# yhg926/MetaKSSD

Hardware: AMD Instinct MI355X
Metric: Gbases/s sketched (150 bp synthetic reads, L3K11 -A) (higher is better)
Workload: dtype u64 k-mers over u8 bases (integer)

## Files before the change

### metakssd_amd/csrc/mk_engine.hip

```cpp
#include "metakssd_hip.h"
#include "mk_poison.hip.h"
#include "mk_kernels.hip.h"
#include "mk_stream.hip.h"
#include "mk_fastq_long.hip.h"
#include "mk_batch.hip.h"
#include "mk_gz.hip.h"
#include "mk_packed.hip.h"

#include <math.h>
#include <stdarg.h>
#include <stdio.h>
#include <stdlib.h>
#include <string.h>

#include <vector>

static thread_local char g_create_error[512] = "";

struct mk_evpair { hipEvent_t a, b; };
#define MK_TICKETS 16
#define MK_REGIONS 3
#define MK_REGION_BYTES ((size_t)256 << 20)

struct mk_engine {
// ... 796 lines not shown
  if (e->tail_active) {
    if (e->split_stream && e->stream == e->own_stream) {
      MK_HIP(e, hipEventRecord(e->ev_scan_pre, e->own_stream));
      MK_HIP(e, hipStreamWaitEvent(e->split_stream, e->ev_scan_pre, 0));
      e->stream = e->split_stream;
    }
    e->tail_active = false;
  }
  return MK_OK;
}

extern "C" int mk_sketch_begin_occ(mk_engine *e, int min_occurrence) {
  if (!e) return MK_ERR_ARG;
  if (min_occurrence < 1 || min_occurrence >= 15)
    return mk_fail(e, MK_ERR_ARG, "fastq2co(): Occurence num should be 1..14 (got %d)", min_occurrence);
  int rc = mk_sketch_begin(e, MK_MODE_OCC_SET);
  if (rc == MK_OK) e->min_occ = (uint32_t)min_occurrence;
  return rc;
}

extern "C" int mk_sketch_begin(mk_engine *e, int mode) {
  if (!e) return MK_ERR_ARG;
  const bool tail = (mode & MK_BEGIN_NOTHING_FOLLOWS) != 0;
  mode &= ~MK_BEGIN_NOTHING_FOLLOWS;
  if (mode < MK_MODE_KOC || mode > MK_MODE_OCC_SET) return MK_ERR_ARG;
  MK_HIP(e, hipSetDevice(e->device));
  { int rc = mk_tables_alloc(e); if (rc) return rc; }
  { int rc = mk_tail_end(e); if (rc) return rc; }
  e->tail = tail && e->scan_stream && e->stream == e->split_stream;
  { int rc = mk_poison_scratch(e); if (rc) return rc; }
  mk_evpair ev{};
  if (e->profiling) { ev = mk_ev_get(e); MK_HIP(e, hipEventRecord(ev.a, e->stream)); }
  bool clear_front = false;
  if (e->sparse && e->tables_tracked) {
    if (!e->tab.fr || e->big_maybe_dirty) {
      hipLaunchKernelGGL(mk_dirty_list_kernel, dim3(1), dim3(1024), 0, e->stream, e->d_dirty_acc, e->acc_words, e->d_list_acc, e->d_nlist, 1,
                         (const uint32_t *)nullptr);
      hipLaunchKernelGGL(mk_dirty_clear_kernel, dim3((unsigned)e->num_cu * 8u), dim3(256), 0, e->stream, e->tab.kc, e->tab.ordinv, e->kp.S,
                         (const uint32_t *)e->d_list_acc, (const uint32_t *)e->d_nlist, (uint32_t)MK_SPARSE_SHIFT, (uint32_t *)nullptr,
                         (const uint32_t *)nullptr, (const uint32_t *)nullptr, (uint32_t)MK_DUMP_SHIFT);
      MK_HIP(e, hipGetLastError());
    }
    if (e->tab.fr) { clear_front = true; e->big_maybe_dirty = false; }
    if (!e->slot_clean) {
      MK_HIP(e, hipMemsetAsync(e->d_slot, 0xFF, (size_t)e->kp.S * sizeof(uint32_t), e->stream));
      e->slot_clean = true;
    }
  } else {
    if (!e->tab.fr || e->big_maybe_dirty) MK_HIP(e, hipMemsetAsync(e->d_tab, 0, e->tab_bytes, e->stream));
    if (e->tab.fr) { clear_front = true; e->big_maybe_dirty = false; }
    if (e->sparse) {
      MK_HIP(e, hipMemsetAsync(e->d_slot, 0xFF, (size_t)e->kp.S * sizeof(uint32_t), e->stream));
      MK_HIP(e, hipMemsetAsync(e->d_dirty_acc, 0, (size_t)e->acc_words * 4, e->stream));
      MK_HIP(e, hipMemsetAsync(e->d_dirty_slot, 0, (size_t)e->slot_words * 4, e->stream));
      e->tables_tracked = true;
      e->slot_clean = true;
    }
  }
  {
    const unsigned long long n16 = clear_front ? (unsigned long long)e->front_slots : 0ull;
    unsigned long long blocks = (n16 + 1023u) / 1024u;
    if (blocks > (unsigned long long)e->num_cu * 8u) blocks = (unsigned long long)e->num_cu * 8u;
    if (blocks == 0) blocks = 1;
    const bool fa = e->fa_used && e->d_fa_state;
    hipLaunchKernelGGL(mk_begin_clear_kernel, dim3((unsigned)blocks), dim3(256), 0, e->stream, (uint4 *)e->d_front, n16, e->d_counters,
                       (uint32_t *)e->d_fa_state, fa ? (uint32_t)(sizeof(mk_fa_state) / 4u) : 0u);
    MK_HIP(e, hipGetLastError());
    e->counter0_used = false;
  }
  if (e->profiling) { MK_HIP(e, hipEventRecord(ev.b, e->stream)); e->ev_clear.push_back(ev); }
  e->region_open = false;
  e->mode = mode;
  e->min_occ = 1;
  e->begun = true;
  e->compacted = false;
  e->count_queued = false;
  e->D = 0;
  e->fa_used = false; e->fa_final = false; e->fa_tail = 0; e->fa_rows_done = 0; e->fa_pitch = 0;
  e->fq_used = false; e->fq_pending = false; e->fq_carry_len = 0; e->fq_total = 0; e->fq_timed = false; e->fq_frame_ms = 0;
  return MK_OK;
}

template <int K, int SK, bool V, int T, int NP, bool OP>
static hipError_t mk_launch_scan_t(mk_engine *e, const mk_scan_args &a, dim3 grid, size_t lds, hipStream_t s) {
  const void *fn = (const void *)mk_scan_kernel<K, SK, V, T, NP, OP>;
  size_t *granted = nullptr;
  for (auto &g : e->lds_granted) if (g.first == fn) granted = &g.second;
  if (!granted) { e->lds_granted.emplace_back(fn, 0); granted = &e->lds_granted.back().second; }
  if (lds > *granted) {
    hipError_t r = hipFuncSetAttribute(fn, hipFuncAttributeMaxDynamicSharedMemorySize, (int)lds);
    if (r != hipSuccess) return r;
    *granted = lds;
  }
  hipLaunchKernelGGL((mk_scan_kernel<K, SK, V, T, NP, OP>), grid, dim3(T), lds, s, a);
  return hipGetLastError();
}
template <int K, int SK, bool V>
static hipError_t mk_launch_scan_k(mk_engine *e, int threads, bool onepass, const mk_scan_args &a, dim3 grid, size_t lds, hipStream_t s) {
  constexpr int NPBIG = V ? MK_MAX_PIECES : MK_MAX_CB / 4;
  constexpr int NPSMALL = V ? 5 : 20;
  const bool small = a.ppr <= (uint32_t)NPSMALL;
  if constexpr (V) {
    if (onepass && small)
      return threads >= 1024 ? mk_launch_scan_t<K, SK, V, 1024, NPSMALL, true>(e, a, grid, lds, s)
             : threads >= 768 ? mk_launch_scan_t<K, SK, V, 768, NPSMALL, true>(e, a, grid, lds, s)
                              : mk_launch_scan_t<K, SK, V, 512, NPSMALL, true>(e, a, grid, lds, s);
  }
  switch (threads) {
    case 1024: return small ? mk_launch_scan_t<K, SK, V, 1024, NPSMALL, false>(e, a, grid, lds, s) : mk_launch_scan_t<K, SK, V, 1024, NPBIG, false>(e, a, grid, lds, s);
    case 768: return small ? mk_launch_scan_t<K, SK, V, 768, NPSMALL, false>(e, a, grid, lds, s) : mk_launch_scan_t<K, SK, V, 768, NPBIG, false>(e, a, grid, lds, s);
    default: return small ? mk_launch_scan_t<K, SK, V, 512, NPSMALL, false>(e, a, grid, lds, s) : mk_launch_scan_t<K, SK, V, 512, NPBIG, false>(e, a, grid, lds, s);
  }
}

static int mk_launch_scan_ex(mk_engine *e, const uint8_t *rows_dev, uint32_t stride, uint32_t pitch, uint32_t rowlen, uint64_t nreads,
                             const unsigned long long *nreads_dev, uint64_t first_ord) {
  if (nreads == 0) return MK_OK;
  if (nreads >= (1ull << 31)) return mk_fail(e, MK_ERR_ARG, "scan launch of %llu reads: the caller splits pushes below 2^31", (unsigned long long)nreads);
  const bool wide = (stride & MK_ROWS_WIDE) != 0;
  const bool packed = (stride & (MK_ROWS_PACKED | MK_ROWS_WIDE)) != 0;
  if (packed) { stride &= ~(MK_ROWS_PACKED | MK_ROWS_WIDE); pitch = stride; }
  mk_scan_args a{};
  a.rows = rows_dev; a.nreads = nreads; a.first_ord = first_ord; a.stride = stride;
  a.pitch = pitch; a.rowlen = rowlen; a.nreads_dev = nreads_dev;
  const bool vec = (stride % 16u == 0) && (pitch % 16u == 0) && (((uintptr_t)rows_dev & 15u) == 0);
  const bool tuned_sk = (e->P.subk == 6 && e->P.k >= 9 && e->P.k <= 11) || (e->P.subk == 5 && e->P.k == 11);
  const bool tuned_geom = tuned_sk && stride % 8u == 0;
  const uint32_t g = vec ? 16u : (tuned_geom ? 8u : 4u);
  const uint32_t max_cb = e->tune_cb;
  a.ncb = (stride + max_cb - 1) / max_cb;
  a.CB = ((stride + a.ncb - 1) / a.ncb + g - 1) / g * g;
  if (a.CB > max_cb) { a.ncb++; a.CB = ((stride + a.ncb - 1) / a.ncb + g - 1) / g * g; }
  a.ncb = (stride + a.CB - 1) / a.CB;
  a.ppr = a.CB / (vec ? 16u : 4u);
  a.ppr_inv = (1u << 20) / a.ppr + 1u;
  a.rowdw = (a.CB / 4u) | 1u;
  a.wave_lds_dwords = ((64u * a.rowdw + 1u) & ~1u) + 2u;
  a.bm_words = 1u << e->bm_bits;
  const int tuned_k = (tuned_sk && stride % 8u == 0 && a.CB % 8u == 0) ? e->P.k : 0;
  if (packed && !tuned_k) return mk_fail(e, MK_ERR_ARG, "packed rows need a geometry with a tuned scan kernel");
  a.mt_words = tuned_k && e->P.subk == 6 ? MK_ZMASK_WORDS : 0u;
  a.pair_subk = tuned_k ? (uint32_t)e->P.subk : 0u;
  if (tuned_k && e->P.subk == 5) a.bm_words = 16384u;
  a.dimmask = (uint32_t)((1ull << (4 * e->P.subk)) - 1ull);
  a.accept = e->d_accept; a.n_accept = e->n_accept;
  a.shuf = e->d_shuf;
  a.accept_bits = e->d_accept_bits;
  a.kp = e->kp;
  a.tab = e->tab;
  a.cand = e->d_cand; a.cand_count = e->d_cand_count; a.cand_cap = e->cand_cap;
  a.batch = e->cur_batch;
  if (a.batch) a.tab.fr = nullptr;
  const bool onepass = e->tune_onepass && vec && a.ncb == 2 && stride == 2u * a.CB && a.ppr <= 5u;
  int threads = e->tune_threads;
  size_t lds = 0;
  const size_t fwords = tuned_k && e->P.subk == 6 && !packed ? (size_t)MK_ZF_WORDS : (size_t)a.bm_words;
  for (;; threads -= 256) {
    lds = ((size_t)a.mt_words + fwords + (size_t)(threads / 64) * a.wave_lds_dwords) * 4u;
    if (vec) lds += 2u * (a.ppr <= 5u ? 5u : (uint32_t)MK_MAX_PIECES) * 64u * 4u;
    if (packed) { threads = 1024; lds = ((size_t)a.mt_words + (size_t)a.bm_words) * 4u; }
    if (lds <= 160u * 1024u || threads <= 512) break;
  }
  if (lds > 160u * 1024u) return mk_fail(e, MK_ERR_ARG, "scan: LDS budget exceeded (%zu bytes)", lds);
  const uint32_t waves = (uint32_t)threads / 64u;
  const uint64_t ntiles = (nreads + 63) / 64;
  uint64_t blocks = (ntiles + waves - 1) / waves;
  uint64_t wgs_per_cu = 1;
#ifdef MK_TUNING
  if (const char *t = getenv("MK_SCAN_WGS_PER_CU")) { const int v = atoi(t); if (v >= 1 && v * waves <= 16u) wgs_per_cu = (uint64_t)v; }
#endif
  const uint64_t scan_cus = e->scan_stream ? (uint64_t)e->scan_cus : (uint64_t)e->num_cu;
  if (blocks > scan_cus * wgs_per_cu) blocks = scan_cus * wgs_per_cu;
  dim3 grid((unsigned)blocks);
#ifdef MK_TUNING
  if (getenv("MK_DEBUG")) {
    static int once = 0;
    if (!once++) fprintf(stderr, "scan cfg: threads %d blocks %llu CB %u ncb %u rowdw %u lds %zu B onepass %d\n", threads,
                         (unsigned long long)blocks, a.CB, a.ncb, a.rowdw, lds, (int)onepass);
  }
#endif

  if (!a.batch) e->big_maybe_dirty = true;
  hipStream_t ss = e->stream;
  if (e->scan_stream) {
    MK_HIP(e, hipEventRecord(e->ev_scan_pre, e->stream));
    MK_HIP(e, hipStreamWaitEvent(e->scan_stream, e->ev_scan_pre, 0));
    ss = e->scan_stream;
  }
  mk_evpair ev{};
  if (e->profiling) { ev = mk_ev_get(e); MK_HIP(e, hipEventRecord(ev.a, ss)); }
  hipError_t r;
  if (packed) {
    auto launch_packed = [&](auto kern) -> hipError_t {
      const void *fn = (const void *)kern;
      size_t *granted = nullptr;
      for (auto &g : e->lds_granted) if (g.first == fn) granted = &g.second;
      if (!granted) { e->lds_granted.emplace_back(fn, 0); granted = &e->lds_granted.back().second; }
      if (lds > *granted) {
        const hipError_t rr = hipFuncSetAttribute(fn, hipFuncAttributeMaxDynamicSharedMemorySize, (int)lds);
        if (rr != hipSuccess) return rr;
        *granted = lds;
      }
      hipLaunchKernelGGL(kern, grid, dim3(1024), lds, ss, a);
      return hipGetLastError();
    };
    if (wide) switch (tuned_k * 10 + e->P.subk) {
      case 116: r = launch_packed(mk_scan_packed_kernel<11, 6, true>); break;
      case 106: r = launch_packed(mk_scan_packed_kernel<10, 6, true>); break;
      case 96: r = launch_packed(mk_scan_packed_kernel<9, 6, true>); break;
      default: r = launch_packed(mk_scan_packed_kernel<11, 5, true>); break;
    } else switch (tuned_k * 10 + e->P.subk) {
      case 116: r = launch_packed(mk_scan_packed_kernel<11, 6>); break;
      case 106: r = launch_packed(mk_scan_packed_kernel<10, 6>); break;
      case 96: r = launch_packed(mk_scan_packed_kernel<9, 6>); break;
      default: r = launch_packed(mk_scan_packed_kernel<11, 5>); break;
    }
  } else
  switch (tuned_k * 10 + (tuned_k ? e->P.subk : 0)) {
    case 116: r = vec ? mk_launch_scan_k<11, 6, true>(e, threads, onepass, a, grid, lds, ss) : mk_launch_scan_k<11, 6, false>(e, threads, false, a, grid, lds, ss); break;
    case 106: r = vec ? mk_launch_scan_k<10, 6, true>(e, threads, onepass, a, grid, lds, ss) : mk_launch_scan_k<10, 6, false>(e, threads, false, a, grid, lds, ss); break;
    case 96: r = vec ? mk_launch_scan_k<9, 6, true>(e, threads, onepass, a, grid, lds, ss) : mk_launch_scan_k<9, 6, false>(e, threads, false, a, grid, lds, ss); break;
    case 115: r = vec ? mk_launch_scan_k<11, 5, true>(e, threads, onepass, a, grid, lds, ss) : mk_launch_scan_k<11, 5, false>(e, threads, false, a, grid, lds, ss); break;
    default: r = vec ? mk_launch_scan_k<0, 0, true>(e, threads, onepass, a, grid, lds, ss) : mk_launch_scan_k<0, 0, false>(e, threads, false, a, grid, lds, ss); break;
  }
  if (r != hipSuccess) return mk_fail(e, MK_ERR_HIP, "scan launch: %s", hipGetErrorString(r));
  if (e->profiling) {
    MK_HIP(e, hipEventRecord(ev.b, ss));
    e->ev_scan.push_back(ev);
    e->prof_rows += nreads;
    e->prof_bytes += nreads * stride;
  }
  if (e->scan_stream) {
    MK_HIP(e, hipEventRecord(e->ev_scan_post, ss));
    if (e->tail && e->begun && !a.batch && e->stream == e->split_stream) {
      MK_HIP(e, hipEventRecord(e->ev_scan_pre, e->split_stream));
      MK_HIP(e, hipStreamWaitEvent(e->own_stream, e->ev_scan_pre, 0));
      e->stream = e->own_stream;
      e->tail_active = true;
    }
    MK_HIP(e, hipStreamWaitEvent(e->stream, e->ev_scan_post, 0));
  }
  {
    const uint32_t used_slots = (uint32_t)blocks * waves;
    mk_evpair ev2{};
    if (e->profiling) { ev2 = mk_ev_get(e); MK_HIP(e, hipEventRecord(ev2.a, e->stream)); }
    const uint32_t rwgs = (used_slots + MK_RESOLVE_THREADS / 64 - 1) / (MK_RESOLVE_THREADS / 64);
    const uint32_t rcus = e->scan_stream && e->stream == e->split_stream ? (uint32_t)e->split_cus : (uint32_t)e->num_cu;
    uint32_t rgrid = rwgs < rcus ? rwgs : rcus;
#ifdef MK_TUNING
    if (const char *t = getenv("MK_RESOLVE_GRID")) { const uint32_t g = (uint32_t)atoi(t); if (g && g <= used_slots) rgrid = g; }
#endif
    const size_t rlds = (size_t)a.bm_words * 4u + (size_t)(MK_RESOLVE_THREADS / 64) * 2u * MK_RQ_CAP * sizeof(uint4);
    {
      const void *fn = (const void *)mk_resolve_kernel;
      size_t *granted = nullptr;
      for (auto &g : e->lds_granted) if (g.first == fn) granted = &g.second;
      if (!granted) { e->lds_granted.emplace_back(fn, 0); granted = &e->lds_granted.back().second; }
      if (rlds > *granted) {
        MK_HIP(e, hipFuncSetAttribute(fn, hipFuncAttributeMaxDynamicSharedMemorySize, (int)rlds));
        *granted = rlds;
      }
    }
    hipLaunchKernelGGL(mk_resolve_kernel, dim3(rgrid), dim3(MK_RESOLVE_THREADS), rlds, e->stream, a, used_slots);
    MK_HIP(e, hipGetLastError());
#ifdef MK_TUNING
    if (getenv("MK_COUNT_RECORDS")) {
      static int shown = 0;
      if (shown++ < 3) {
        std::vector<uint32_t> h(used_slots);
        MK_HIP(e, hipStreamSynchronize(e->stream));
        MK_HIP(e, hipMemcpy(h.data(), e->d_cand_count, (size_t)used_slots * 4, hipMemcpyDeviceToHost));
        unsigned long long sum = 0;
        for (uint32_t v : h) sum += v;
        fprintf(stderr, "[scan records] %llu reads -> %llu candidate records (%.4f a read, %.3f %% of the 8-base windows of 150-base reads)\n",
                (unsigned long long)nreads, sum, (double)sum / (double)nreads, 100.0 * (double)sum / ((double)nreads * 19.0));
      }
    }
#endif
    if (e->profiling) { MK_HIP(e, hipEventRecord(ev2.b, e->stream)); e->ev_resolve.push_back(ev2); }
  }
  if (!a.batch) { e->compacted = false; e->count_queued = false; }
  return MK_OK;
}

static int mk_launch_scan(mk_engine *e, const uint8_t *rows_dev, uint32_t stride, uint64_t nreads, uint64_t first_ord) {
  return mk_launch_scan_ex(e, rows_dev, stride, stride, 0u, nreads, nullptr, first_ord);
}

static int mk_check_push(mk_engine *e, const void *rows, uint32_t stride) {
  if (!e) return MK_ERR_ARG;
  if (!e->begun) return mk_fail(e, MK_ERR_STATE, "push before mk_sketch_begin");
  if (stride & MK_ROWS_PACKED) {
    if (stride != (MK_PACKED_PITCH | MK_ROWS_PACKED)) return mk_fail(e, MK_ERR_ARG, "push: packed rows have a pitch of %u bytes", MK_PACKED_PITCH);
    if (!mk_params_packed_ok(&e->P)) return mk_fail(e, MK_ERR_ARG, "push: packed rows need a geometry with a tuned scan kernel (mk_params_packed_ok)");
    if (!rows) return mk_fail(e, MK_ERR_ARG, "push: rows == NULL");
    if ((uintptr_t)rows & 15u) return mk_fail(e, MK_ERR_ARG, "push: packed rows must be 16-byte aligned");
    return MK_OK;
  }
  if (!rows || stride < 4 || stride > 4096 || (stride & 3u)) return mk_fail(e, MK_ERR_ARG, "push: stride must be a multiple of 4 in 4..4096");
  return MK_OK;
}

extern "C" int mk_sketch_push_reads_device(mk_engine *e, const uint8_t *rows_dev, uint32_t stride, uint64_t nreads,
                                           uint64_t first_read_ordinal) {
  int rc = mk_check_push(e, rows_dev, stride);
  if (rc) return rc;
  MK_HIP(e, hipSetDevice(e->device));
  if ((first_read_ordinal + nreads) >> 51) return mk_fail(e, MK_ERR_ARG, "read ordinal too large");
  const uint64_t waves = (uint64_t)e->num_cu * (uint64_t)(e->tune_threads / 64);
  uint64_t per = (uint64_t)(e->cand_cap / 32u) * 64u * waves;
  if (per < 64u * waves) per = 64u * waves;
  if (per > (1ull << 30)) per = 1ull << 30;
// ... 1538 lines not shown
```

### metakssd_amd/csrc/mk_kernels.hip.h

```cpp
#pragma once
#include <hip/hip_runtime.h>
#include <stdint.h>

#include "host/mk_host_internal.h"
#include "mk_key.hip.h"

#define MK_WAVE 64
#define MK_MAX_CB 128
#define MK_MAX_PIECES 8
#define MK_EMPTY32 0xFFFFFFFFu
#define MK_ZMASK_WORDS 256u
#define MK_CNT_BITS 24
#define MK_CNT_MASK 0xFFFFFFull
#define MK_CNT_SAT 0xF00000ull

struct mk_table {
  unsigned long long *kc;
  unsigned long long *ordinv;
  uint32_t *err;
  uint32_t *dirty;
  uint32_t dirty_shift;
  const struct mk_front *fr;
};
struct mk_front {
// ... 304 lines not shown
      }
      hits &= (0xFFu << jmin) & ~(0xFFFFFFFFu << e);
    }
    if (__any(hits != 0u)) {
      const uint32_t pos0 = (r.y & 0x1FFu) << 3, h2 = r.z & 0xFFFFu, h3 = r.z >> 16;
      const uint64_t ord0 = ((a.first_ord + (uint64_t)r.w) << 12) | pos0;
      do {
        const bool has = hits != 0u;
        const uint32_t j = has ? (uint32_t)__builtin_ctz(hits) : 0u;
        hits &= hits - 1u;
        const uint32_t dd = 2u * (j + 1u);
        const uint32_t fl = __builtin_amdgcn_alignbit(r.x, lo, 30u - 2u * j);
        const uint32_t fhi = ((h3 << dd) | (h2 >> (16u - dd))) & hm;
        const uint64_t ord = ord0 + j;
        mk_wring_push(r1, has, make_uint4(fl, fhi, (uint32_t)ord, (uint32_t)(ord >> 32)));
        mk_wave_lds_fence();
        drain1(64u);
      } while (__any(hits != 0u));
    }
  };

  uint4 r[MK_RESOLVE_UNROLL], rn[MK_RESOLVE_UNROLL];
  bool more = fetch(r);
  while (more) {
    more = fetch(rn);
#pragma unroll
    for (uint32_t u = 0; u < MK_RESOLVE_UNROLL; u++) process(r[u]);
#pragma unroll
    for (uint32_t u = 0; u < MK_RESOLVE_UNROLL; u++) r[u] = rn[u];
  }
  mk_wave_lds_fence();
  drain1(1u);
  drain2(1u);
  if (a.tab.fr) {
    if (lane == 0 && installed) atomicAdd(&wg_installed, installed);
    __syncthreads();
    if (threadIdx.x == 0) mk_front_launch_end(a.tab, wg_installed, gridDim.x);
  }
}

__device__ __forceinline__ uint32_t mk_filter_mask(uint32_t x) {
  return (1u << (x & 31u)) | (1u << ((x >> 2) & 31u)) | (1u << ((x >> 6) & 31u));
}

template <int K>
struct mk_kmer {
  uint64_t f;
  __device__ __forceinline__ void reset() { f = 0; }
  __device__ __forceinline__ void roll(uint32_t code, const mk_keyparams &kp) { f = ((f << 2) | code) & kp.tupmask; }
  __device__ __forceinline__ uint64_t fwd() const { return f; }
  __device__ __forceinline__ uint32_t dimx(const mk_keyparams &kp, uint32_t dimmask) const { return (uint32_t)(f >> kp.out2) & dimmask; }
  static __device__ __forceinline__ uint32_t TL(const mk_keyparams &kp) { return kp.TL; }
};

template <int K>
struct mk_kmer_hi {
  static_assert(K > 8 && K <= 16, "two-half representation needs 32 < 4K <= 64");
  static constexpr uint32_t HMASK = (uint32_t)((1ull << (4 * K - 32)) - 1ull);
  uint32_t flo, fhi;
  __device__ __forceinline__ void reset() { flo = fhi = 0; }
  __device__ __forceinline__ void roll(uint32_t code, const mk_keyparams &) {
    const uint32_t nfhi = __builtin_amdgcn_alignbit(fhi, flo, 30) & HMASK;
    flo = (flo << 2) | code;
    fhi = nfhi;
  }
  __device__ __forceinline__ uint64_t fwd() const { return ((uint64_t)fhi << 32) | flo; }
  __device__ __forceinline__ uint32_t dimx(const mk_keyparams &kp, uint32_t dimmask) const {
    return (uint32_t)(fwd() >> kp.out2) & dimmask;
  }
  static __device__ __forceinline__ uint32_t TL(const mk_keyparams &) { return 2u * K; }
};
template <> struct mk_kmer<9> : mk_kmer_hi<9> {};
template <> struct mk_kmer<10> : mk_kmer_hi<10> {};
template <> struct mk_kmer<11> : mk_kmer_hi<11> {};
template <> struct mk_kmer<12> : mk_kmer_hi<12> {};



template <int J>
__device__ __forceinline__ uint32_t mk_code_of(uint32_t w) {
  uint32_t r;
  asm("v_bfe_u32 %0, %1, %2, 2" : "=v"(r) : "v"(w), "n"(8 * J + 1));
  return r;
}

template <uint32_t SH>
__device__ __forceinline__ uint32_t mk_onehot_at(uint32_t flo) {
  if constexpr (SH == 8u) {
    uint32_t r;
    asm("v_lshlrev_b32_sdwa %0, %1, %2 dst_sel:DWORD dst_unused:UNUSED_PAD src0_sel:BYTE_1 src1_sel:DWORD"
        : "=v"(r) : "v"(flo), "s"(1u));
    return r;
  } else {
    return 1u << ((flo >> SH) & 31u);
  }
}

__device__ __forceinline__ uint32_t mk_nonzero_bytes(uint32_t v) {
  return (((v & 0x7F7F7F7Fu) + 0x7F7F7F7Fu) | v) & 0x80808080u;
}

__device__ __forceinline__ uint32_t mk_zmask(uint32_t b) {
  uint32_t m = 0, h = b * 0x9E3779B1u + 0x7F4A7C15u;
  while (__builtin_popcount(m) < 6) {
    m |= 1u << (h >> 27);
    h = h * 0x85EBCA6Bu + 0xC2B2AE35u;
  }
  return m;
}
#define MK_ZF_WORDS 16384u
__device__ __forceinline__ void mk_build_zfilter(uint32_t *masktab, uint32_t *bitmap, const mk_scan_args &a) {
  for (uint32_t i = threadIdx.x; i < MK_ZMASK_WORDS; i += blockDim.x) masktab[i] = mk_zmask(i);
  for (uint32_t i = threadIdx.x; i < MK_ZF_WORDS; i += blockDim.x) bitmap[i] = 0u;
  __syncthreads();
  for (uint32_t i = threadIdx.x; i < a.n_accept; i += blockDim.x) {
    const uint32_t d = (uint32_t)mk_scan_to_ref_codes(a.accept[i]);
    const uint32_t z1 = d & 0x3FFFFFu, z2 = d >> 2;
    atomicOr(&bitmap[(z1 >> 8) & (MK_ZF_WORDS - 1u)], masktab[z1 & 255u]);
    atomicOr(&bitmap[(z2 >> 8) & (MK_ZF_WORDS - 1u)], masktab[z2 & 255u]);
  }
  __syncthreads();
}

__device__ __forceinline__ void mk_build_xfilter(uint32_t *bitmap, const mk_scan_args &a) {
  for (uint32_t i = threadIdx.x; i < 16384u; i += blockDim.x) bitmap[i] = 0u;
  __syncthreads();
  for (uint32_t i = threadIdx.x; i < a.n_accept; i += blockDim.x) {
    const uint32_t d = (uint32_t)mk_scan_to_ref_codes(a.accept[i]) & 0xFFFFFu;
    atomicOr(&bitmap[d >> 6], 1u << (d & 31u));
  }
  __syncthreads();
}

__device__ __forceinline__ void mk_build_filter(uint32_t *bitmap, const mk_scan_args &a) {
  for (uint32_t i = threadIdx.x; i < a.bm_words; i += blockDim.x) bitmap[i] = 0u;
  __syncthreads();
  for (uint32_t i = threadIdx.x; i < a.n_accept; i += blockDim.x) {
    const uint32_t d = (uint32_t)mk_scan_to_ref_codes(a.accept[i]);
    atomicOr(&bitmap[(d >> 10) & (a.bm_words - 1u)], mk_filter_mask(d));
  }
  __syncthreads();
}

template <int K, int SUBK, bool VEC16, int THREADS, int NPIECES, bool ONEPASS>
__global__ void __launch_bounds__(THREADS) mk_scan_kernel(const mk_scan_args a) {
  static_assert(K == 0 || SUBK == 6 || (SUBK == 5 && K == 11), "tuned instantiations: k 9..11 with subk 6, k 11 with subk 5");
  extern __shared__ __align__(16) uint32_t lds[];
  constexpr uint32_t WAVES = THREADS / 64;
  const uint32_t lane = threadIdx.x & 63u, wave = threadIdx.x >> 6;
  const uint32_t fwords = (K != 0 && SUBK == 6) ? MK_ZF_WORDS : a.bm_words;
  uint32_t *bitmap = lds + a.mt_words;
  uint32_t *tile = lds + a.mt_words + fwords + wave * a.wave_lds_dwords;

  if constexpr (VEC16) {
    if (wave == 0) {
      uint32_t *t = lds + a.mt_words + fwords + WAVES * a.wave_lds_dwords + lane;
#pragma unroll
      for (int i = 0; i < NPIECES; i++) {
        const uint32_t q = lane + 64u * i;
        const uint32_t r = (q * a.ppr_inv) >> 20, c = q - r * a.ppr;
        t[128 * i] = r * a.pitch + c * 16u;
        t[128 * i + 64] = r * a.rowdw + c * 4u;
      }
    }
  }
  if constexpr (K != 0 && SUBK == 6) mk_build_zfilter(lds, bitmap, a);
  else if constexpr (K != 0) mk_build_xfilter(bitmap, a);
  else mk_build_filter(bitmap, a);

  const uint32_t filter_base = (uint32_t)(uintptr_t)(mk_lds_cu32)bitmap;
  constexpr uint32_t MTW = (K != 0 && SUBK == 6) ? MK_ZMASK_WORDS : 0u;
  if (K != 0 && (filter_base != MTW * 4u || a.mt_words != MTW || a.bm_words != 16384u || a.dimmask != (SUBK == 6 ? 0xFFFFFFu : 0xFFFFFu))) {
    if (threadIdx.x == 0) atomicOr(&a.tab.err[0], 4u);
    if (lane == 0) a.cand_count[blockIdx.x * WAVES + wave] = 0u;
    return;
  }
  const mk_scan_args *ka = (const mk_scan_args *)__builtin_amdgcn_kernarg_segment_ptr();
  const uint32_t TL = mk_kmer<K>::TL(a.kp);
  const uint32_t dimmask = a.dimmask;
  const uint32_t wmask4 = (a.bm_words - 1u) << 2;
  uint64_t nreads = a.nreads;
  if (a.nreads_dev) { const uint64_t nd = *a.nreads_dev; if (nd < nreads) nreads = nd; }
  const uint32_t ntiles = (uint32_t)((nreads + 63u) >> 6);
  const uint32_t wave_global = blockIdx.x * WAVES + wave;
  const uint32_t nwaves = gridDim.x * WAVES;
  uint4 *const my_cand = a.cand + (size_t)__builtin_amdgcn_readfirstlane(wave_global) * a.cand_cap;
  if (wave_global >= ntiles) {
    if (lane == 0) a.cand_count[wave_global] = 0u;
    return;
  }

  using piece_t = typename std::conditional<VEC16, uint4, uint32_t>::type;
  constexpr int NP = NPIECES;
  constexpr uint32_t PW = VEC16 ? 16u : 4u;
  piece_t regs[NP];
  piece_t regs2[ONEPASS ? NP : 1];
  auto goff_calc = [&](int i) { const uint32_t q = lane + 64u * i; const uint32_t r = (q * a.ppr_inv) >> 20, c = q - r * a.ppr; return r * a.pitch + c * PW; };
  auto loff_calc = [&](int i) { const uint32_t q = lane + 64u * i; const uint32_t r = (q * a.ppr_inv) >> 20, c = q - r * a.ppr; return r * a.rowdw + c * (PW / 4u); };
  const uint32_t *offtab = lds + a.mt_words + fwords + WAVES * a.wave_lds_dwords + lane;
  auto goff_of = [&](int i) { if constexpr (VEC16) return offtab[128 * i]; else return goff_calc(i); };
  auto loff_of = [&](int i) { if constexpr (VEC16) return offtab[128 * i + 64]; else return loff_calc(i); };
  auto issue_loads = [&](uint32_t tile_id, uint32_t cb) {
    const uint32_t row0 = tile_id << 6;
    const uint8_t *base = a.rows + (uint64_t)row0 * a.pitch + (uint64_t)cb * a.CB;
    const uint32_t cols_here = min(a.CB, a.stride - cb * a.CB);
    if constexpr (ONEPASS) {
      if (row0 + 64u <= nreads) {
#pragma unroll
        for (int i = 0; i < NP; i++)
          if ((uint32_t)i < a.ppr) { regs[i] = *(const piece_t *)(base + goff_of(i)); regs2[i] = *(const piece_t *)(base + a.CB + goff_of(i)); }
      } else {
        const uint32_t rows_here = (uint32_t)(nreads - row0);
#pragma unroll
        for (int i = 0; i < NP; i++) {
          if ((uint32_t)i < a.ppr) {
            const uint32_t q = lane + 64u * i;
            const uint32_t r = (q * a.ppr_inv) >> 20;
            if (r < rows_here) { regs[i] = *(const piece_t *)(base + goff_of(i)); regs2[i] = *(const piece_t *)(base + a.CB + goff_of(i)); }
          }
        }
      }
    } else if (row0 + 64u <= nreads && cols_here == a.CB) {
#pragma unroll
      for (int i = 0; i < NP; i++)
        if ((uint32_t)i < a.ppr) regs[i] = *(const piece_t *)(base + goff_of(i));
    } else {
      const uint32_t rows_here = (uint32_t)(nreads - row0 < 64u ? nreads - row0 : 64u);
#pragma unroll
      for (int i = 0; i < NP; i++) {
        if ((uint32_t)i < a.ppr) {
          const uint32_t q = lane + 64u * i;
          const uint32_t r = (q * a.ppr_inv) >> 20, c = q - r * a.ppr;
          if (r < rows_here && c * PW < cols_here) regs[i] = *(const piece_t *)(base + goff_of(i));
        }
      }
    }
  };
  auto commit = [&](uint32_t cb) {
    (void)cb;
#pragma unroll
    for (int i = 0; i < NP; i++) {
      if ((uint32_t)i < a.ppr) {
        if constexpr (VEC16) {
          uint32_t *p = tile + loff_of(i);
          if constexpr (ONEPASS) {
            const piece_t v = cb ? regs2[i] : regs[i];
            p[0] = v.x; p[1] = v.y; p[2] = v.z; p[3] = v.w;
          } else {
            p[0] = regs[i].x; p[1] = regs[i].y; p[2] = regs[i].z; p[3] = regs[i].w;
          }
        } else {
          tile[loff_of(i)] = regs[i];
        }
      }
    }
  };

  mk_kmer<K> km;
  km.reset();
  uint32_t hh = 0;
  uint32_t run = 0;
  bool done = true;
  uint32_t qn = 0;
  const uint32_t *myrow = tile + lane * a.rowdw;
  uint64_t ord_row = 0;

  struct quad { uint64_t u0, u1, u2, u3; uint32_t m0, m1, m2, m3, w0, w1, w2, w3; };

  auto lookup = [&](uint32_t &mask, uint32_t &word) {
    const uint32_t xx = km.dimx(a.kp, dimmask);
    if constexpr (K != 0) {
      const uint32_t z = xx & 0x3FFFFFu;
      word = *(mk_lds_cu32)(uintptr_t)(((z >> 6) & (SUBK == 6 ? (MK_ZF_WORDS - 1u) << 2 : wmask4)) + filter_base);
      mask = lds[z & 255u];
    } else {
      word = *(mk_lds_cu32)(uintptr_t)(((xx >> 8) & wmask4) + filter_base);
      mask = mk_filter_mask(xx);
    }
  };
  auto push_record = [&](bool hit, const uint4 r) {
    const uint64_t m = __ballot(hit);
    if (m == 0) return;
    const uint32_t cnt = (uint32_t)__popcll(m);
    if (qn + cnt > a.cand_cap) {
      mk_resolve_inline(ka, hit, r, K != 0 ? nullptr : bitmap);
      return;
    }
    if (hit) my_cand[qn + mk_mbcnt(m)] = r;
    qn = __builtin_amdgcn_readfirstlane(qn + cnt);
  };
  auto push_pair = [&](const bool hit, const uint64_t hm, const uint4 r) {
    const uint32_t cnt = (uint32_t)__popcll(hm);
    if (qn + cnt > a.cand_cap) { mk_resolve_inline(ka, hit, r, nullptr); return; }
    if (hit) *(uint4 *)((uint8_t *)my_cand + (qn + mk_mbcnt(hm)) * 16u) = r;
    qn += cnt;
  };
  auto push = [&](bool hit, uint64_t fwd, uint32_t pos) {
    const uint64_t ord = ord_row | (uint64_t)pos;
    push_record(hit, make_uint4((uint32_t)fwd, (uint32_t)(fwd >> 32), (uint32_t)ord, (uint32_t)(ord >> 32) | 0x80000000u));
  };

  auto fast4 = [&](uint32_t codes, quad &q) {
    km.roll(codes & 3u, a.kp);         q.u0 = km.fwd(); lookup(q.m0, q.w0);
    km.roll((codes >> 8) & 3u, a.kp);  q.u1 = km.fwd(); lookup(q.m1, q.w1);
    km.roll((codes >> 16) & 3u, a.kp); q.u2 = km.fwd(); lookup(q.m2, q.w2);
    km.roll(codes >> 24, a.kp);        q.u3 = km.fwd(); lookup(q.m3, q.w3);
  };
  auto general4 = [&](uint32_t w, uint32_t codes, uint32_t x, quad &q) {
    auto one = [&](uint32_t j, uint64_t &pu, uint32_t &pm, uint32_t &pw) {
      const uint32_t ch = (w >> (8u * j)) & 0xffu;
      const bool valid = ((x >> (8u * j)) & 0xffu) == 0u;
      if (!done && ch == '\n') done = true;
      const bool ok = valid && !done;
      if (ok) { km.roll((codes >> (8u * j)) & 3u, a.kp); run++; }
      else if (!done) run = 0;
      pu = km.fwd();
      lookup(pm, pw);
      if (!(ok && run >= TL)) { pm = 1u; pw = 0u; }
    };
    one(0, q.u0, q.m0, q.w0); one(1, q.u1, q.m1, q.w1); one(2, q.u2, q.m2, q.w2); one(3, q.u3, q.m3, q.w3);
  };
  auto hits4 = [&](const quad &q, uint32_t pos0) {
    push((q.m0 & ~q.w0) == 0u, q.u0, pos0);
    push((q.m1 & ~q.w1) == 0u, q.u1, pos0 + 1u);
    push((q.m2 & ~q.w2) == 0u, q.u2, pos0 + 2u);
    push((q.m3 & ~q.w3) == 0u, q.u3, pos0 + 3u);
  };
  auto resolve4 = [&](const quad &q, uint32_t pos0) {
    const uint32_t t0 = q.m0 & ~q.w0, t1 = q.m1 & ~q.w1, t2 = q.m2 & ~q.w2, t3 = q.m3 & ~q.w3;
    const uint32_t mn = min(min(t0, t1), min(t2, t3));
    if (__any(mn == 0u)) hits4(q, pos0);
  };
  auto decode = [&](uint32_t w, uint32_t &codes, uint32_t &x) {
    codes = (w >> 1) & 0x03030303u;
    const uint32_t expect = __builtin_amdgcn_perm(0u, 0x47544341u, codes);
    x = (w & 0xDFDFDFDFu) ^ expect;
  };
  auto slow_dword = [&](uint32_t w, uint32_t codes, uint32_t x, uint32_t pos0) {
    if (__all(x == 0u && !done && run + 4u < TL)) {
      km.roll(codes & 3u, a.kp); km.roll((codes >> 8) & 3u, a.kp); km.roll((codes >> 16) & 3u, a.kp); km.roll(codes >> 24, a.kp);
      run += 4u;
      return;
    }
    const uint32_t inval = mk_nonzero_bytes(x);
    const uint32_t notnl = mk_nonzero_bytes(w ^ 0x0A0A0A0Au);
    const uint32_t pat = inval | (notnl >> 1);
    const uint32_t pat0 = __builtin_amdgcn_readfirstlane(pat), run0 = __builtin_amdgcn_readfirstlane(run);
    if (__all(pat == pat0 && run == run0 && !done)) {
      uint32_t urun = run0;
#pragma unroll 1
      for (uint32_t j = 0; j < 4; j++) {
        if (!(pat0 & (0x40u << (8u * j)))) { done = true; break; }
        if (pat0 & (0x80u << (8u * j))) { urun = 0; continue; }
        km.roll((codes >> (8u * j)) & 3u, a.kp);
        urun++;
        if (urun >= TL) {
          uint32_t m, wd;
          lookup(m, wd);
          push((m & ~wd) == 0u, km.fwd(), pos0 + j);
        }
      }
      run = urun;
      return;
    }
    quad q;
    general4(w, codes, x, q);
    resolve4(q, pos0);
  };

  uint32_t nt_tile = wave_global;
  uint32_t nt_cb = 0;
  issue_loads(nt_tile, nt_cb);
  for (uint32_t tile_id = wave_global; tile_id < ntiles; tile_id += nwaves) {
    const uint32_t row0 = tile_id << 6;
    km.reset(); run = 0; hh = 0;
    done = row0 + lane >= nreads;
    ord_row = (a.first_ord + row0 + lane) << 12;
    for (uint32_t cb = 0; cb < a.ncb; cb++) {
      mk_wave_lds_fence();
      commit(cb);
      mk_wave_lds_fence();
      if (a.rowlen) {
        const uint32_t c0b = cb * a.CB;
        if (a.rowlen >= c0b && a.rowlen < c0b + a.CB) {
          uint32_t *q = tile + lane * a.rowdw + ((a.rowlen - c0b) >> 2);
          const uint32_t sh = (a.rowlen & 3u) * 8u;
          *q = (*q & ((1u << sh) - 1u)) | (0x0A0A0A0Au << sh);
        }
        mk_wave_lds_fence();
      }
      if constexpr (ONEPASS) {
        if (cb == 1u) { nt_tile += nwaves; if (nt_tile < ntiles) issue_loads(nt_tile, 0u); }
      } else {
        if (++nt_cb == a.ncb) { nt_cb = 0; nt_tile += nwaves; }
        if (nt_tile < ntiles) issue_loads(nt_tile, nt_cb);
      }
      if (__all(done)) continue;

      const uint32_t col0 = cb * a.CB;
      const uint32_t ndw = min(a.CB, a.stride - col0) >> 2;
      const uint32_t npairs = ndw >> 1;
      if constexpr (K != 0) {
        constexpr uint32_t SH = 2u * (K - SUBK) - 2u;
        constexpr uint32_t HM = mk_kmer<K>::HMASK;
        static_assert(SH + 4u * SUBK <= 32u, "inner substring must lie inside flo(j-1)");
        constexpr uint32_t D = SUBK == 6 ? (SH - 2u) / 2u : 1u;
        static_assert(SUBK != 6 || (SH >= 4u && SH <= 8u), "pair probing: z[0..7] at bits 2..9 of a low word D bases earlier");
        static_assert(SUBK != 5 || SH == 10u, "per-base probing: word address in WORD_1 of before_{j+1}, bit index in BYTE_1 of before_{j-1}");
        uint32_t urun = 0;
        auto in_step = [&]() -> bool {
          const uint32_t rc = min(run, TL);
          urun = __builtin_amdgcn_readlane(rc, (int)__builtin_ctzll(~__ballot(done) & __builtin_amdgcn_read_exec()));
          return __all(done || rc == urun);
        };
        bool step = in_step();
        uint32_t nw0 = myrow[0], nw1 = myrow[1];
        uint32_t p = 0;
        uint32_t flo = km.flo;
        uint32_t pa[3] = {0u, 0u, 0u};
        auto oh_init = [&]() {
          if constexpr (SUBK == 6) {
#pragma unroll
            for (uint32_t k = 0; k < D; k++) pa[k] = (flo >> (2u * (D - k))) & 0x3FCu;
          } else {
            pa[0] = flo >> 2;
          }
        };
        oh_init();
        uint32_t w0, w1, c0, x0, c1, x1;
        auto next_pair = [&]() {
          w0 = nw0; w1 = nw1;
          nw0 = myrow[2 * p + 2];
          nw1 = myrow[2 * p + 3];
          decode(w0, c0, x0);
          decode(w1, c1, x1);
        };
        auto pair_body = [&](const bool rollonly, const uint32_t jmin, const uint32_t e, const bool live, const uint64_t livem) {
          const uint32_t fstart = flo;
          const uint32_t lo = __builtin_amdgcn_perm(__builtin_amdgcn_udot4(c0, 0x01041040u, 0u, false),
                                                    __builtin_amdgcn_udot4(c1, 0x01041040u, 0u, false), 0x04000C0Cu);
          if (rollonly) {
            flo = __builtin_amdgcn_alignbit(fstart, lo, 16);
            oh_init();
          } else {
            const uint32_t f0 = __builtin_amdgcn_alignbit(fstart, lo, 30), f1 = __builtin_amdgcn_alignbit(fstart, lo, 28);
            const uint32_t f2 = __builtin_amdgcn_alignbit(fstart, lo, 26), f3 = __builtin_amdgcn_alignbit(fstart, lo, 24);
            const uint32_t f4 = __builtin_amdgcn_alignbit(fstart, lo, 22), f5 = __builtin_amdgcn_alignbit(fstart, lo, 20);
            const uint32_t f6 = __builtin_amdgcn_alignbit(fstart, lo, 18), f7 = __builtin_amdgcn_alignbit(fstart, lo, 16);
            const uint32_t bj[9] = {fstart, f0, f1, f2, f3, f4, f5, f6, f7};
            bool fired;
            if constexpr (SUBK == 6) {
              uint32_t mm[4], dd[4];
#pragma unroll
              for (uint32_t t = 0; t < 4; t++) {
                const uint32_t wsrc = bj[2u * t + 1u];
                dd[t] = *(mk_lds_cu32)(uintptr_t)(((wsrc >> (SH + 8u)) & ((MK_ZF_WORDS - 1u) << 2)) + MK_ZMASK_WORDS * 4u);
                mm[t] = *(mk_lds_cu32)(uintptr_t)(2u * t >= D ? bj[2u * t - D] & 0x3FCu : pa[2u * t]);
              }
#pragma unroll
              for (uint32_t k = 0; k < D; k++) pa[k] = bj[8u - D + k] & 0x3FCu;
              flo = f7;
              __builtin_amdgcn_sched_barrier(0);
              __builtin_amdgcn_s_waitcnt(0xC07F);
              const uint32_t tt0 = mm[0] & ~dd[0], tt1 = mm[1] & ~dd[1], tt2 = mm[2] & ~dd[2], tt3 = mm[3] & ~dd[3];
              fired = min(min(tt0, tt1), min(tt2, tt3)) == 0u;
            } else {
              uint32_t wd[8];
#pragma unroll
              for (uint32_t j = 0; j < 8; j++) {
                uint32_t addr;
                asm("v_and_b32_sdwa %0, %1, %2 dst_sel:DWORD dst_unused:UNUSED_PAD src0_sel:WORD_1 src1_sel:DWORD"
                    : "=v"(addr) : "v"(bj[j + 1u]), "v"(0xFFFCu));
                wd[j] = *(mk_lds_cu32)(uintptr_t)addr;
              }
              const uint32_t bprev = pa[0];
              pa[0] = f6;
              flo = f7;
              __builtin_amdgcn_sched_barrier(0);
              __builtin_amdgcn_s_waitcnt(0xC07F);
              uint32_t sh[8];
#pragma unroll
              for (uint32_t j = 0; j < 8; j++) {
                const uint32_t src = j == 0 ? bprev : bj[j - 1u];
                asm("v_lshrrev_b32_sdwa %0, %1, %2 dst_sel:DWORD dst_unused:UNUSED_PAD src0_sel:BYTE_1 src1_sel:DWORD"
                    : "=v"(sh[j]) : "v"(src), "v"(wd[j]));
              }
              fired = (((sh[0] | sh[1] | sh[2]) | (sh[3] | sh[4] | sh[5]) | (sh[6] | sh[7])) & 1u) != 0u;
            }
            const bool hit = fired && live;
            const uint64_t hm = __builtin_amdgcn_ballot_w64(fired) & livem;
            if (hm) {
              const uint32_t meta = ((col0 + 8u * p) >> 3) | (jmin << 9) | (e << 12);
              push_pair(hit, hm, make_uint4(fstart, (lo & 0xFFFF0000u) | meta, hh, (uint32_t)(row0 + lane)));
            }
          }
          hh = __builtin_amdgcn_perm(hh, fstart, 0x05040100u);
          ++p;
        };
        uint64_t donem = __ballot(done);
        for (;;) {
          if (step) {
            bool left = false, more = true;
            auto pair_is_bases = [&]() -> bool {
              const uint64_t bad = ((uint64_t)x1 << 32) | x0;
              uint64_t lanes_ok;
              asm("v_cmp_eq_u64_e64 %0, 0, %1" : "=s"(lanes_ok) : "v"(bad));
              return (lanes_ok | donem) == __builtin_amdgcn_read_exec();
            };
            while (urun + 1u < TL) {
              next_pair();
              if (!pair_is_bases()) { left = true; break; }
              pair_body(urun + 8u < TL, TL - 1u - urun, 8u, !done, ~donem);
              urun += 8u;
              if (p == npairs) { more = false; break; }
            }
            if (!left && more) {
              const uint32_t p0 = p;
              for (;;) {
                next_pair();
                if (!pair_is_bases()) { left = true; break; }
                pair_body(false, 0u, 8u, !done, ~donem);
                if (p == npairs) break;
              }
              urun += 8u * (p - p0);
            }
            run = urun;
            if (!left) break;
          } else {
            next_pair();
          }
          {
            const uint64_t inval = ((uint64_t)mk_nonzero_bytes(x1) << 32) | mk_nonzero_bytes(x0);
            const uint64_t nl = ((uint64_t)(mk_nonzero_bytes(w1 ^ 0x0A0A0A0Au) ^ 0x80808080u) << 32) |
                                (mk_nonzero_bytes(w0 ^ 0x0A0A0A0Au) ^ 0x80808080u);
            const uint32_t e = inval ? (uint32_t)__builtin_ctzll(inval) >> 3 : 8u;
            const uint32_t jm = run + 1u >= TL ? 0u : TL - 1u - run;
            const bool say = !done && jm < e;
            pair_body(false, jm & 7u, e, say, __builtin_amdgcn_ballot_w64(say));
            run = inval ? (uint32_t)__builtin_clzll(inval) >> 3 : min(run + 8u, 0xFFFFu);
            done = done || nl != 0ull;
            donem = __ballot(done);
            if (donem == __builtin_amdgcn_read_exec() || p == npairs) break;
            step = in_step();
          }
        }
        km.flo = flo;
        km.fhi = (hh >> 16) & HM;
      } else {
        uint32_t nw0 = myrow[0], nw1 = ndw > 1 ? myrow[1] : 0x0a0a0a0au;
        for (uint32_t p = 0; p < npairs; p++) {
          const uint32_t w0 = nw0, w1 = nw1;
          if (p + 1 < npairs) { nw0 = myrow[2 * p + 2]; nw1 = myrow[2 * p + 3]; }
          else if (ndw & 1u) nw0 = myrow[ndw - 1];
          uint32_t c0, x0, c1, x1;
          decode(w0, c0, x0);
          decode(w1, c1, x1);
          const uint32_t pos0 = col0 + 8u * p;
          if (__all((x0 | x1) == 0u && !done && run + 1u >= TL)) {
            quad qa, qb;
            fast4(c0, qa);
            fast4(c1, qb);
            run += 8u;
            resolve4(qa, pos0);
            resolve4(qb, pos0 + 4u);
          } else {
            slow_dword(w0, c0, x0, pos0);
            slow_dword(w1, c1, x1, pos0 + 4u);
            if (__all(done)) break;
          }
        }
        if ((ndw & 1u) && !__all(done)) {
          uint32_t c0, x0;
          decode(nw0, c0, x0);
          slow_dword(nw0, c0, x0, col0 + 4u * (ndw - 1u));
        }
      }
    }
  }
  if (lane == 0) a.cand_count[wave_global] = qn;
}

__global__ void __launch_bounds__(1024) mk_import_kernel(mk_table tab, uint32_t S, const unsigned long long *keys,
                                                         const uint32_t *counts, const unsigned long long *ords, uint64_t n) {
  __shared__ uint32_t wg_installed;
  if (threadIdx.x == 0) wg_installed = 0u;
  __syncthreads();
  const bool front_open = mk_front_open(tab);
  uint32_t installed = 0;
  for (uint64_t i = (uint64_t)blockIdx.x * blockDim.x + threadIdx.x; i < n; i += (uint64_t)gridDim.x * blockDim.x)
    installed += mk_upsert(tab, S, keys[i], ords[i], counts[i], front_open) ? 1u : 0u;
  if (tab.fr) {
    if (installed) atomicAdd(&wg_installed, installed);
    __syncthreads();
    if (threadIdx.x == 0) mk_front_launch_end(tab, wg_installed, gridDim.x);
  }
}

__global__ void __launch_bounds__(1024) mk_front_fold_kernel(mk_table tab, uint32_t S) {
  const mk_front f = *tab.fr;
  if (__hip_atomic_load(&f.state[1], __ATOMIC_RELAXED, __HIP_MEMORY_SCOPE_AGENT) == 0u) return;
  const uint64_t slots = (uint64_t)f.mask + 1u;
  for (uint64_t i = (uint64_t)blockIdx.x * blockDim.x + threadIdx.x; i < slots; i += (uint64_t)gridDim.x * blockDim.x) {
    const unsigned long long kc = f.kc1[i];
    if (kc == 0ull) continue;
    const uint32_t c = (uint32_t)(kc & MK_CNT_MASK);
    mk_upsert_big(tab, S, kc >> MK_CNT_BITS, ~f.ordinv1[i], c > 65535u ? 65535u : c);
    f.kc1[i] = 0ull;
    f.ordinv1[i] = 0ull;
  }
}

struct mk_dist {
  unsigned long long *key;
  unsigned long long *ord;
  uint32_t *cnt;
  uint64_t cap;
};

#define MK_SPLIT_MAX 16u
__global__ void __launch_bounds__(1024) mk_split_count_kernel(mk_dist d, const unsigned long long *Dp, uint32_t nparts, unsigned long long *hist) {
  __shared__ uint32_t h[MK_SPLIT_MAX];
  if (threadIdx.x < MK_SPLIT_MAX) h[threadIdx.x] = 0u;
  __syncthreads();
  const uint64_t D = *Dp;
  for (uint64_t i = (uint64_t)blockIdx.x * blockDim.x + threadIdx.x; i < D; i += (uint64_t)gridDim.x * blockDim.x)
    atomicAdd(&h[(uint32_t)(d.key[i] % nparts)], 1u);
  __syncthreads();
  if (threadIdx.x < nparts && h[threadIdx.x]) atomicAdd(&hist[threadIdx.x], (unsigned long long)h[threadIdx.x]);
}
__global__ void mk_split_offsets_kernel(const unsigned long long *hist, unsigned long long *cursor, uint32_t nparts) {
  unsigned long long at = 0;
  for (uint32_t g = 0; g < nparts; g++) { cursor[g] = at; at += hist[g]; }
}
__global__ void __launch_bounds__(1024) mk_split_scatter_kernel(mk_dist d, const unsigned long long *Dp, uint32_t nparts, unsigned long long *cursor,
                                                                unsigned long long *okey, uint32_t *ocnt, unsigned long long *oord, uint64_t ocap) {
  __shared__ uint32_t h[MK_SPLIT_MAX];
  __shared__ unsigned long long base[MK_SPLIT_MAX];
  const uint64_t D = *Dp;
  const uint64_t tiles = (D + blockDim.x - 1) / blockDim.x;
  for (uint64_t t = blockIdx.x; t < tiles; t += gridDim.x) {
    if (threadIdx.x < MK_SPLIT_MAX) h[threadIdx.x] = 0u;
    __syncthreads();
    const uint64_t i = t * blockDim.x + threadIdx.x;
    unsigned long long k = 0;
    uint32_t g = 0, r = 0;
    if (i < D) { k = d.key[i]; g = (uint32_t)(k % nparts); r = atomicAdd(&h[g], 1u); }
    __syncthreads();
    if (threadIdx.x < nparts) base[threadIdx.x] = h[threadIdx.x] ? atomicAdd(&cursor[threadIdx.x], (unsigned long long)h[threadIdx.x]) : 0ull;
    __syncthreads();
    if (i < D) {
      const unsigned long long o = base[g] + r;
      if (o < ocap) { okey[o] = k; ocnt[o] = d.cnt[i]; oord[o] = d.ord[i]; }
    }
    __syncthreads();
  }
}
__global__ void mk_set_counter_kernel(unsigned long long *counter, unsigned long long v) { counter[0] = v; }


__global__ void __launch_bounds__(1024) mk_dirty_list_kernel(uint32_t *bitmap, uint32_t nwords, uint32_t *list, uint32_t *count,
                                                            int clear_bitmap, const uint32_t *big_used) {
  if (big_used && __hip_atomic_load(big_used, __ATOMIC_RELAXED, __HIP_MEMORY_SCOPE_AGENT) == 0u) {
    if (threadIdx.x == 0) *count = 0u;
    return;
  }
  __shared__ uint32_t base_s;
  if (threadIdx.x == 0) base_s = 0;
  __syncthreads();
  for (uint32_t w0 = 0; w0 < nwords; w0 += 1024u) {
    const uint32_t w = w0 + threadIdx.x;
    uint32_t bits = w < nwords ? bitmap[w] : 0u;
    if (bits && clear_bitmap) bitmap[w] = 0u;
    uint32_t off = bits ? atomicAdd(&base_s, (uint32_t)__popc(bits)) : 0u;
    while (bits) {
      list[off++] = (w << 5) + (uint32_t)__builtin_ctz(bits);
// ... 504 lines not shown
```

Baseline: 3063.

## Use unpadded 16-byte tile rows and a two-pair software-pipelined scan loop

For onepass tuned-k scans, rows in each wave's LDS tile are now stored unpadded, so each lane writes and reads whole uint4 chunks. The LDS offset table half is dropped. The steady-state inner loop handles two 8-base pairs per iteration, loads 16 bytes at a time, and interleaves the filter LDS lookups of one window with the address computation of the next, using sched barriers and explicit waitcnt. The aim is fewer LDS instructions and hidden LDS latency in the hot loop. The cost is possible LDS bank conflicts from the unpadded row stride and much more complex control flow.

```diff
diff --git a/metakssd_amd/csrc/mk_engine.hip b/metakssd_amd/csrc/mk_engine.hip
--- a/metakssd_amd/csrc/mk_engine.hip
+++ b/metakssd_amd/csrc/mk_engine.hip
@@ -972,12 +972,14 @@
   a.batch = e->cur_batch;
   if (a.batch) a.tab.fr = nullptr;
   const bool onepass = e->tune_onepass && vec && a.ncb == 2 && stride == 2u * a.CB && a.ppr <= 5u;
+  const bool tile16 = onepass && tuned_k && !packed;
+  if (tile16) { a.rowdw = a.CB / 4u; a.wave_lds_dwords = 64u * a.rowdw + 4u; }
   int threads = e->tune_threads;
   size_t lds = 0;
   const size_t fwords = tuned_k && e->P.subk == 6 && !packed ? (size_t)MK_ZF_WORDS : (size_t)a.bm_words;
   for (;; threads -= 256) {
     lds = ((size_t)a.mt_words + fwords + (size_t)(threads / 64) * a.wave_lds_dwords) * 4u;
-    if (vec) lds += 2u * (a.ppr <= 5u ? 5u : (uint32_t)MK_MAX_PIECES) * 64u * 4u;
+    if (vec) lds += (tile16 ? 1u : 2u) * (a.ppr <= 5u ? 5u : (uint32_t)MK_MAX_PIECES) * 64u * 4u;
     if (packed) { threads = 1024; lds = ((size_t)a.mt_words + (size_t)a.bm_words) * 4u; }
     if (lds <= 160u * 1024u || threads <= 512) break;
   }
diff --git a/metakssd_amd/csrc/mk_kernels.hip.h b/metakssd_amd/csrc/mk_kernels.hip.h
--- a/metakssd_amd/csrc/mk_kernels.hip.h
+++ b/metakssd_amd/csrc/mk_kernels.hip.h
@@ -480,6 +480,8 @@
   uint32_t *bitmap = lds + a.mt_words;
   uint32_t *tile = lds + a.mt_words + fwords + wave * a.wave_lds_dwords;
 
+  constexpr bool T16 = ONEPASS && K != 0;
+  constexpr uint32_t OTS = T16 ? 64u : 128u;
   if constexpr (VEC16) {
     if (wave == 0) {
       uint32_t *t = lds + a.mt_words + fwords + WAVES * a.wave_lds_dwords + lane;
@@ -487,8 +489,8 @@
       for (int i = 0; i < NPIECES; i++) {
         const uint32_t q = lane + 64u * i;
         const uint32_t r = (q * a.ppr_inv) >> 20, c = q - r * a.ppr;
-        t[128 * i] = r * a.pitch + c * 16u;
-        t[128 * i + 64] = r * a.rowdw + c * 4u;
+        t[OTS * i] = r * a.pitch + c * 16u;
+        if constexpr (!T16) t[128 * i + 64] = r * a.rowdw + c * 4u;
       }
     }
   }
@@ -498,7 +500,8 @@
 
   const uint32_t filter_base = (uint32_t)(uintptr_t)(mk_lds_cu32)bitmap;
   constexpr uint32_t MTW = (K != 0 && SUBK == 6) ? MK_ZMASK_WORDS : 0u;
-  if (K != 0 && (filter_base != MTW * 4u || a.mt_words != MTW || a.bm_words != 16384u || a.dimmask != (SUBK == 6 ? 0xFFFFFFu : 0xFFFFFu))) {
+  if (K != 0 && (filter_base != MTW * 4u || a.mt_words != MTW || a.bm_words != 16384u || a.dimmask != (SUBK == 6 ? 0xFFFFFFu : 0xFFFFFu) ||
+                 (T16 && (a.rowdw * 4u != a.CB || (a.wave_lds_dwords & 3u) != 0u || a.wave_lds_dwords < 64u * a.rowdw + 4u)))) {
     if (threadIdx.x == 0) atomicOr(&a.tab.err[0], 4u);
     if (lane == 0) a.cand_count[blockIdx.x * WAVES + wave] = 0u;
     return;
@@ -526,7 +529,7 @@
   auto goff_calc = [&](int i) { const uint32_t q = lane + 64u * i; const uint32_t r = (q * a.ppr_inv) >> 20, c = q - r * a.ppr; return r * a.pitch + c * PW; };
   auto loff_calc = [&](int i) { const uint32_t q = lane + 64u * i; const uint32_t r = (q * a.ppr_inv) >> 20, c = q - r * a.ppr; return r * a.rowdw + c * (PW / 4u); };
   const uint32_t *offtab = lds + a.mt_words + fwords + WAVES * a.wave_lds_dwords + lane;
-  auto goff_of = [&](int i) { if constexpr (VEC16) return offtab[128 * i]; else return goff_calc(i); };
+  auto goff_of = [&](int i) { if constexpr (VEC16) return offtab[OTS * i]; else return goff_calc(i); };
   auto loff_of = [&](int i) { if constexpr (VEC16) return offtab[128 * i + 64]; else return loff_calc(i); };
   auto issue_loads = [&](uint32_t tile_id, uint32_t cb) {
     const uint32_t row0 = tile_id << 6;
@@ -569,7 +572,10 @@
 #pragma unroll
     for (int i = 0; i < NP; i++) {
       if ((uint32_t)i < a.ppr) {
-        if constexpr (VEC16) {
+        if constexpr (T16) {
+          const piece_t v = cb ? regs2[i] : regs[i];
+          *(uint4 *)(tile + 4u * lane + 256u * i) = make_uint4(v.x, v.y, v.z, v.w);
+        } else if constexpr (VEC16) {
           uint32_t *p = tile + loff_of(i);
           if constexpr (ONEPASS) {
             const piece_t v = cb ? regs2[i] : regs[i];
@@ -742,7 +748,10 @@
           return __all(done || rc == urun);
         };
         bool step = in_step();
-        uint32_t nw0 = myrow[0], nw1 = myrow[1];
+        uint32_t nw0 = 0, nw1 = 0;
+        uint4 nq = make_uint4(0u, 0u, 0u, 0u);
+        if constexpr (T16) nq = *(const uint4 *)myrow;
+        else { nw0 = myrow[0]; nw1 = myrow[1]; }
         uint32_t p = 0;
         uint32_t flo = km.flo;
         uint32_t pa[3] = {0u, 0u, 0u};
@@ -757,9 +766,18 @@
         oh_init();
         uint32_t w0, w1, c0, x0, c1, x1;
         auto next_pair = [&]() {
-          w0 = nw0; w1 = nw1;
-          nw0 = myrow[2 * p + 2];
-          nw1 = myrow[2 * p + 3];
+          if constexpr (T16) {
+            if (p & 1u) {
+              w0 = nq.z; w1 = nq.w;
+              nq = *(const uint4 *)(myrow + 2 * p + 2);
+            } else {
+              w0 = nq.x; w1 = nq.y;
+            }
+          } else {
+            w0 = nw0; w1 = nw1;
+            nw0 = myrow[2 * p + 2];
+            nw1 = myrow[2 * p + 3];
+          }
           decode(w0, c0, x0);
           decode(w1, c1, x1);
         };
@@ -844,11 +862,97 @@
             }
             if (!left && more) {
               const uint32_t p0 = p;
-              for (;;) {
-                next_pair();
-                if (!pair_is_bases()) { left = true; break; }
-                pair_body(false, 0u, 8u, !done, ~donem);
-                if (p == npairs) break;
+              if constexpr (T16) {
+                if (p & 1u) {
+                  next_pair();
+                  if (!pair_is_bases()) left = true;
+                  else { pair_body(false, 0u, 8u, !done, ~donem); more = p != npairs; }
+                }
+                if constexpr (SUBK == 6) {
+                  uint32_t c2, c3;
+                  auto decode_step = [&]() -> bool {
+                    uint32_t x2, x3;
+                    w0 = nq.x; w1 = nq.y;
+                    decode(w0, c0, x0);
+                    decode(w1, c1, x1);
+                    decode(nq.z, c2, x2);
+                    decode(nq.w, c3, x3);
+                    const uint32_t bad = (x0 | x1 | x2) | x3;
+                    return (__builtin_amdgcn_ballot_w64(bad == 0u) | donem) == __builtin_amdgcn_read_exec();
+                  };
+                  auto lo_of = [&](const uint32_t ca, const uint32_t cb_) {
+                    return __builtin_amdgcn_perm(__builtin_amdgcn_udot4(ca, 0x01041040u, 0u, false), __builtin_amdgcn_udot4(cb_, 0x01041040u, 0u, false), 0x04000C0Cu);
+                  };
+                  auto win_addr = [&](const uint32_t fs, const uint32_t lo, const uint32_t (&pin)[3], uint32_t (&ad)[4], uint32_t (&am)[4], uint32_t (&pout)[3], uint32_t &fend) {
+                    const uint32_t bj[9] = {fs, __builtin_amdgcn_alignbit(fs, lo, 30), __builtin_amdgcn_alignbit(fs, lo, 28), __builtin_amdgcn_alignbit(fs, lo, 26),
+                                            __builtin_amdgcn_alignbit(fs, lo, 24), __builtin_amdgcn_alignbit(fs, lo, 22), __builtin_amdgcn_alignbit(fs, lo, 20),
+                                            __builtin_amdgcn_alignbit(fs, lo, 18), __builtin_amdgcn_alignbit(fs, lo, 16)};
+#pragma unroll
+                    for (uint32_t t = 0; t < 4; t++) {
+                      ad[t] = (bj[2u * t + 1u] >> (SH + 8u)) & ((MK_ZF_WORDS - 1u) << 2);
+                      am[t] = 2u * t >= D ? bj[2u * t - D] & 0x3FCu : pin[2u * t];
+                    }
+#pragma unroll
+                    for (uint32_t k = 0; k < 3; k++) pout[k] = k < D ? bj[8u - D + k] & 0x3FCu : 0u;
+                    fend = bj[8];
+                  };
+                  auto window_hits = [&](const uint32_t (&mm)[4], const uint32_t (&dd)[4], const uint32_t fs, const uint32_t lo) {
+                    const uint32_t tt0 = mm[0] & ~dd[0], tt1 = mm[1] & ~dd[1], tt2 = mm[2] & ~dd[2], tt3 = mm[3] & ~dd[3];
+                    const bool fired = min(min(tt0, tt1), min(tt2, tt3)) == 0u;
+                    const uint64_t hm = __builtin_amdgcn_ballot_w64(fired) & ~donem;
+                    if (hm) push_pair(fired && !done, hm, make_uint4(fs, (lo & 0xFFFF0000u) | ((col0 + 8u * p) >> 3) | (8u << 12), hh, (uint32_t)(row0 + lane)));
+                    hh = __builtin_amdgcn_perm(hh, fs, 0x05040100u);
+                    ++p;
+                  };
+                  if (!left && more) {
+                    if (decode_step()) for (;;) {
+                      nq = *(const uint4 *)(myrow + 2 * p + 4);
+                      uint32_t ad[4], am[4], mm[4], dd[4], pb[3], f7a, f7b;
+                      const uint32_t lo1 = lo_of(c0, c1);
+                      win_addr(flo, lo1, pa, ad, am, pb, f7a);
+#pragma unroll
+                      for (uint32_t t = 0; t < 4; t++) { dd[t] = *(mk_lds_cu32)(uintptr_t)(ad[t] + MK_ZMASK_WORDS * 4u); mm[t] = *(mk_lds_cu32)(uintptr_t)am[t]; }
+                      __builtin_amdgcn_sched_barrier(0);
+                      const uint32_t lo2 = lo_of(c2, c3);
+                      win_addr(f7a, lo2, pb, ad, am, pa, f7b);
+                      asm volatile("" : "+v"(ad[0]), "+v"(ad[1]), "+v"(ad[2]), "+v"(ad[3]), "+v"(am[0]), "+v"(am[1]), "+v"(am[2]), "+v"(am[3]), "+v"(f7b));
+                      __builtin_amdgcn_sched_barrier(0);
+                      __builtin_amdgcn_s_waitcnt(0xC07F);
+                      window_hits(mm, dd, flo, lo1);
+#pragma unroll
+                      for (uint32_t t = 0; t < 4; t++) { dd[t] = *(mk_lds_cu32)(uintptr_t)(ad[t] + MK_ZMASK_WORDS * 4u); mm[t] = *(mk_lds_cu32)(uintptr_t)am[t]; }
+                      __builtin_amdgcn_sched_barrier(0);
+                      const bool bases = decode_step();
+                      __builtin_amdgcn_sched_barrier(0);
+                      __builtin_amdgcn_s_waitcnt(0xC07F);
+                      window_hits(mm, dd, f7a, lo2);
+                      flo = f7b;
+                      if (p == npairs || !bases) break;
+                    }
+                    left = p != npairs;
+                  }
+                } else if (!left && more) for (;;) {
+                  uint32_t c2, x2, c3, x3;
+                  w0 = nq.x; w1 = nq.y;
+                  decode(w0, c0, x0);
+                  decode(w1, c1, x1);
+                  decode(nq.z, c2, x2);
+                  decode(nq.w, c3, x3);
+                  const uint32_t bad = (x0 | x1 | x2) | x3;
+                  if ((__builtin_amdgcn_ballot_w64(bad == 0u) | donem) != __builtin_amdgcn_read_exec()) { left = true; break; }
+                  nq = *(const uint4 *)(myrow + 2 * p + 4);
+                  pair_body(false, 0u, 8u, !done, ~donem);
+                  c0 = c2; c1 = c3;
+                  pair_body(false, 0u, 8u, !done, ~donem);
+                  if (p == npairs) break;
+                }
+              } else {
+                for (;;) {
+                  next_pair();
+                  if (!pair_is_bases()) { left = true; break; }
+                  pair_body(false, 0u, 8u, !done, ~donem);
+                  if (p == npairs) break;
+                }
               }
               urun += 8u * (p - p0);
             }
```

Measured after the change: 2796. -8.7%, worse.
